# supranational/sppark

Measured on AMD Instinct MI355X. Metric: MSM points/sec (BLS12-381 G1, 2^26 points), higher is better.
Workload: dtype u32

## Files before the change

sppark_amd/csrc/msm/msm_driver.hpp:

```cpp
#pragma once
#include "msm_kernels.hpp"
#include "msm_coop_kernels.hpp"
#include "msm_plan.hpp"
#include "../ec/jacobian_host.hpp"
#include "../util/runtime.hpp"
#include <algorithm>
#include <cmath>
#include <map>
#include <mutex>
#include <vector>

namespace sppark_amd {

template<class FD, class FH, class FRp>
class msm_t {
public:
    typedef FD fp_d;
    static constexpr bool G2_COOP_BUILT = field_is_internal<FD>::value && !field_is_montx<FD>::value;
    typedef mont_dev<FRp> fr_d;
    typedef FH fp_h;
    typedef typename xyzz_dev<fp_d>::mem_t bucket_t;
    typedef jacobian_host<fp_h> point_t;
    static constexpr int STD_WORDS = sizeof(FH) / 4;
    static constexpr size_t FP_BYTES = sizeof(FH);
// ... 248 lines not shown
    {
        if (tune.wbits) return std::min(26u, std::max(8u, tune.wbits));
        unsigned w = 0; double best = 0;
        for (unsigned c = 8; c <= 26; c++) {
            const double cost = (double)((FRp::NBITS - 1) / c + 1) * (double)np + 3.0 * (double)((size_t)1 << (c - 1));
            if (w == 0 || cost < best) { best = cost; w = c; }
        }
        return w;
    }
    void preload(const void* points, size_t np, size_t ffi_affine_sz, bool fixed_base = false)
    {
        HIP_OK(hipSetDevice(gpu->hip_id));
        HIP_OK(hipStreamSynchronize(stream));
        join_default_stream();
        if (np != 0 && (points == nullptr || ffi_affine_sz < 2 * FP_BYTES || np > (1u << 31))) HIP_OK(hipErrorInvalidValue);
        if (np != 0 && fixed_base && !MONTX) HIP_OK(hipErrorNotSupported);
        if (np != 0 && fixed_base && (tune.wbits || np >= FIXED_BASE_MIN)
            && (size_t)((FRp::NBITS - 1) / fixed_base_width(np) + 1) * np >= ((size_t)1 << 31)) HIP_OK(hipErrorInvalidValue);
        if (pre_points) { HIP_OK(hipFree(pre_points)); pre_points = nullptr; pre_n = pre_stride = 0; }
        pre_fb_wbits = pre_fb_nwins = 0;
        if (np == 0) return;
        if (fixed_base && !MONTX) HIP_OK(hipErrorNotSupported);
        if (fixed_base && !tune.wbits && np < FIXED_BASE_MIN) fixed_base = false;
        unsigned fb_w = 0, fb_nw = 1;
        if (fixed_base) {
            fb_w = fixed_base_width(np);
            fb_nw = (FRp::NBITS - 1) / fb_w + 1;
            fb_w = FRp::NBITS / fb_nw + (FRp::NBITS % fb_nw ? 1 : 0);
            if ((size_t)fb_nw * np >= ((size_t)1 << 31)) HIP_OK(hipErrorInvalidValue);
        }
        if (points == nullptr || ffi_affine_sz < 2 * FP_BYTES || np > (1u << 31)) HIP_OK(hipErrorInvalidValue);
        struct dev_buf {
            unsigned char* p = nullptr;
            ~dev_buf() { if (p) (void)hipFree(p); }
        } staging;
        try {
            if constexpr (INTERNAL) {
                const unsigned char* src = (const unsigned char*)points;
                if (!is_device_pointer(points)) {
                    HIP_OK(hipMalloc((void**)&staging.p, np * ffi_affine_sz));
                    HIP_OK(hipMemcpyAsync(staging.p, points, np * ffi_affine_sz, hipMemcpyHostToDevice, stream));
                    src = staging.p;
                }
                HIP_OK(dev_scratch_pool::malloc_or_drain((void**)&pre_points, (size_t)fb_nw * np * conv_stride()));
                launch_convert(pre_points, src, (unsigned)np, ffi_affine_sz);
                if constexpr (MONTX) if (fixed_base) {
                    hipLaunchKernelGGL(k_fixed_base_table<fp_d>, dim3((unsigned)((np + 255) / 256)), dim3(256), 0, stream,
                                       pre_points, (unsigned)np, fb_nw, (unsigned)FRp::NBITS);
                    HIP_OK(hipGetLastError());
                }
            } else {
                HIP_OK(hipMalloc((void**)&pre_points, np * ffi_affine_sz));
                HIP_OK(hipMemcpyAsync(pre_points, points, np * ffi_affine_sz,
                                      is_device_pointer(points) ? hipMemcpyDeviceToDevice : hipMemcpyHostToDevice, stream));
            }
            HIP_OK(hipStreamSynchronize(stream));
        } catch (...) {
            if (pre_points) { (void)hipFree(pre_points); pre_points = nullptr; }
            throw;
        }
        pre_n = np; pre_stride = ffi_affine_sz;
        if (fixed_base) { pre_fb_wbits = fb_w; pre_fb_nwins = fb_nw; }
    }
    unsigned fixed_base_windows() const { return pre_fb_nwins; }
    size_t preloaded() const { return pre_n; }

private:
    void launch_convert(unsigned char* dst, const unsigned char* src, unsigned n, size_t stride, hipStream_t on = nullptr)
    {
        if constexpr (INTERNAL) {
            if (on == nullptr) on = stream;
            unsigned grid = (n + 255) / 256;
            if constexpr (MONTX) {
                if ((stride == 2 * FP_BYTES || stride == 2 * FP_BYTES + 8) && ((size_t)src & 15) == 0 && tune.join != 6) {
                    if (stride == 2 * FP_BYTES) hipLaunchKernelGGL((k_convert_points_staged<fp_d, false>), dim3(grid), dim3(256), 0, on, dst, src, n);
                    else                        hipLaunchKernelGGL((k_convert_points_staged<fp_d, true>), dim3(grid), dim3(256), 0, on, dst, src, n);
                    HIP_OK(hipGetLastError());
                    return;
                }
            }
            if (stride > 2 * FP_BYTES) hipLaunchKernelGGL((k_convert_points<fp_d, true>), dim3(grid), dim3(256), 0, on, dst, src, n, (unsigned)stride);
            else                       hipLaunchKernelGGL((k_convert_points<fp_d, false>), dim3(grid), dim3(256), 0, on, dst, src, n, (unsigned)stride);
            HIP_OK(hipGetLastError());
        }
    }

    size_t choose_chunk(size_t n, size_t stage_per_point) const
    {
        size_t chunk = n;
        if (tune.chunk) chunk = std::min(n, std::max<size_t>(tune.chunk, 1));
        else if (stage_per_point && n > ((size_t)1 << 21)) {
            chunk = std::min<size_t>(std::max<size_t>(n / 4, (size_t)1 << 20), (size_t)1 << 24);
        }
        auto need = [&](size_t c) {
            return make_layout(make_plan(c, FRp::NBITS, tune), true).total + 2 * c * stage_per_point + 1024;
        };
        size_t limit = tune.max_scratch;
        if (!limit) {
            const bool blob_ok = make_layout(make_plan(chunk, FRp::NBITS, tune), true).total <= blob_sz;
            const bool stage_ok = stage_per_point == 0 || 2 * (chunk * stage_per_point + 512) <= stage_sz;
            if (blob_ok && stage_ok) return chunk;
            size_t free_b = 0, total_b = 0;
            if (hipMemGetInfo(&free_b, &total_b) != hipSuccess) { (void)hipGetLastError(); return chunk; }
            limit = free_b - (free_b >> 5) + blob_sz + stage_sz;
        }
        while (need(chunk) > limit && chunk > 4096) chunk = (chunk + 1) / 2;
        return chunk;
    }

    std::vector<size_t> chunk_bounds(size_t n, size_t chunk) const
    {
        std::vector<size_t> b{0};
        for (size_t lo = chunk; lo < n; lo += chunk) b.push_back(lo);
        b.push_back(n);
        return b;
    }

    void sort_group(hipStream_t ss, const msm_plan& p, const layout& l, unsigned b, unsigned w0, unsigned wn,
                    const u32* d_scalars, bool mont, unsigned fb_n = 0, unsigned fb_nwins = 0)
    {
        u32* digits = (u32*)(blob + l.digits[b]);
        u32* sorted = (u32*)(blob + l.sorted[b]);
        u32* H = (u32*)(blob + l.H[b]);
        u32* tot = (u32*)(blob + l.tot[b]);
        u32* off = (u32*)(blob + l.off[b]);
        void* partA = blob + l.partA[b];
        u32* offA = (u32*)(blob + l.offA[b]);
        const bool packed = p.IB != 0;
        unsigned ngp = 1; while (ngp < p.NG) ngp <<= 1;
        const partA_fmt fmt{H, p.IB, p.SH, ngp, p.nslabs};
        const unsigned nlong = p.nbits % p.nwins, sf = nlong == 0 ? wn : (nlong > w0 ? std::min(wn, nlong - w0) : 0u);
        if (fb_n) {
            unsigned grid = std::min<unsigned>((fb_n + 255) / 256, 256 * 16);
            hipLaunchKernelGGL(k_breakdown<fr_d>, dim3(grid), dim3(256), 0, ss,
                               digits, d_scalars, fb_n, fb_nwins, (unsigned)FRp::NBITS, (int)mont, 0u, fb_nwins);
        } else {
            unsigned grid = std::min<unsigned>((p.n + 255) / 256, 256 * 16);
            hipLaunchKernelGGL(k_breakdown<fr_d>, dim3(grid), dim3(256), 0, ss,
                               digits, d_scalars, p.n, p.nwins, p.nbits, (int)mont, w0, wn);
        }
        HIP_OK(hipGetLastError());
        size_t ldsA = (size_t)p.NA * 4, ldsB = ((size_t)1 << p.LB) * 4 + SORT_NT * 4 + (size_t)SORTB_STAGE * 4 + PARTA_MAX_GROUPS * 4;
        if (ldsA > 65536) { lds_attr((const void*)k_histA, ldsA); lds_attr(packed ? (const void*)k_scatterA<true> : (const void*)k_scatterA<false>, ldsA); }
        if (ldsB > 65536) lds_attr(packed ? (const void*)k_sortB<true> : (const void*)k_sortB<false>, ldsB);
        hipLaunchKernelGGL(k_histA, dim3(p.nslabs, wn), dim3(SORT_NT), ldsA, ss,
                           H, digits, p.n, p.nslabs, p.slab_sz, p.NA, p.LB, sf);
        HIP_OK(hipGetLastError());
        size_t na_total = (size_t)wn * p.NA;
        hipLaunchKernelGGL(k_scan_slabs, dim3((unsigned)((na_total + 255) / 256)), dim3(256), 0, ss,
                           H, tot, p.nslabs, p.NA, wn);
        HIP_OK(hipGetLastError());
        hipLaunchKernelGGL(k_scan_parts, dim3(wn), dim3(1024), 0, ss, offA, tot, p.NA);
        HIP_OK(hipGetLastError());
        if (p.NA <= SCATA_MAX_NA && p.LB < 16) {
            const size_t ldsS = scatterA_staged_lds(p.NA);
            lds_attr(packed ? (const void*)k_scatterA_staged<true> : (const void*)k_scatterA_staged<false>, ldsS);
            if (packed) hipLaunchKernelGGL(k_scatterA_staged<true>, dim3(p.nslabs, wn), dim3(SORT_NT), ldsS, ss,
                                           (u32*)partA, digits, H, offA, p.n, p.nslabs, p.slab_sz, p.NA, p.LB, sf, p.IB);
            else        hipLaunchKernelGGL(k_scatterA_staged<false>, dim3(p.nslabs, wn), dim3(SORT_NT), ldsS, ss,
                                           (uint2*)partA, digits, H, offA, p.n, p.nslabs, p.slab_sz, p.NA, p.LB, sf, p.IB);
        } else {
            if (packed) hipLaunchKernelGGL(k_scatterA<true>, dim3(p.nslabs, wn), dim3(SORT_NT), ldsA, ss,
                                           (u32*)partA, digits, H, offA, p.n, p.nslabs, p.slab_sz, p.NA, p.LB, sf, p.IB);
            else        hipLaunchKernelGGL(k_scatterA<false>, dim3(p.nslabs, wn), dim3(SORT_NT), ldsA, ss,
                                           (uint2*)partA, digits, H, offA, p.n, p.nslabs, p.slab_sz, p.NA, p.LB, sf, p.IB);
        }
        HIP_OK(hipGetLastError());
        const unsigned big = tune.big ? tune.big : p.big ? p.big : (1u << 18);
        u32* nbig = (u32*)(blob + l.bigl[b]); u32* blist = nbig + 1; u32* curB = (u32*)(blob + l.curB[b]);
        const bool may_be_big = p.n > big;
        if (may_be_big) HIP_OK(hipMemsetAsync(nbig, 0, 4, ss));
        if (packed) hipLaunchKernelGGL(k_sortB<true>, dim3(p.NA, wn), dim3(SORT_NT), ldsB, ss,
                                       sorted, off, (const u32*)partA, offA, p.n, p.NA, p.LB, sf, big, fmt);
        else        hipLaunchKernelGGL(k_sortB<false>, dim3(p.NA, wn), dim3(SORT_NT), ldsB, ss,
                                       sorted, off, (const uint2*)partA, offA, p.n, p.NA, p.LB, sf, big, fmt);
        HIP_OK(hipGetLastError());
        if (!may_be_big) return;
        hipLaunchKernelGGL(k_big_find, dim3((p.NA * wn + 255) / 256), dim3(256), 0, ss,
                           nbig, blist, off, offA, p.NA, p.LB, sf, wn, big);
        size_t ldsBig = ((size_t)1 << p.LB) * 4;
        const size_t avg = (size_t)p.n / p.NA;
        const unsigned split = avg > big / 2 ? (unsigned)std::min<size_t>(SORTB_SPLIT, avg / (BIG_STAGE / 2) + 1) : SORTB_SPLIT;
        if (packed) hipLaunchKernelGGL(k_big_hist<true>, dim3(1024), dim3(1024), ldsBig, ss, off, (const u32*)partA, offA, nbig, blist, p.n, p.NA, p.LB, sf, split);
        else        hipLaunchKernelGGL(k_big_hist<false>, dim3(1024), dim3(1024), ldsBig, ss, off, (const uint2*)partA, offA, nbig, blist, p.n, p.NA, p.LB, sf, split);
        hipLaunchKernelGGL(k_big_scan, dim3(p.NA > 64 && avg > big / 2 ? 1024 : 64), dim3(1024), 0, ss, off, curB, offA, nbig, blist, p.NA, p.LB, sf);
        const size_t ldsSc = big_scatter_lds(p.LB);
        if (ldsSc > 65536) lds_attr(packed ? (const void*)k_big_scatter<true> : (const void*)k_big_scatter<false>, ldsSc);
        if (packed) hipLaunchKernelGGL(k_big_scatter<true>, dim3(1024), dim3(1024), ldsSc, ss, sorted, curB, (const u32*)partA, offA, nbig, blist, p.n, p.NA, p.LB, sf, split, fmt);
        else        hipLaunchKernelGGL(k_big_scatter<false>, dim3(1024), dim3(1024), ldsSc, ss, sorted, curB, (const uint2*)partA, offA, nbig, blist, p.n, p.NA, p.LB, sf, split, fmt);
        HIP_OK(hipGetLastError());
    }

    void enqueue(const msm_plan& p, const layout& l, const unsigned char* d_points, size_t stride, bool preconverted,
                 const u32* d_scalars, bool mont, std_bucket_t* h_out, bool first_timed, unsigned fb_n = 0, unsigned fb_nwins = 0,
                 bool redo = false, bool may_defer = false)
    {
        const bool flagged = !preconverted && stride > 2 * FP_BYTES;
        const bool multi = p.G > 1;
        if (multi) need_aux();
        if (timing && first_timed && !redo) { need_tev(2 + 2 * p.G); HIP_OK(hipEventRecord(tev[0], stream)); }
        if (multi) {
            HIP_OK(hipEventRecord(ev_fork, stream));
            HIP_OK(hipStreamWaitEvent(aux, ev_fork, 0));
        }
        bucket_t* buckets = (bucket_t*)(blob + l.buckets);
        u32* keyA = (u32*)(blob + l.keyA); bucket_t* ptA = (bucket_t*)(blob + l.ptA);
        u32* keyB = (u32*)(blob + l.keyB); bucket_t* ptB = (bucket_t*)(blob + l.ptB);
        if (multi && !redo) HIP_OK(hipMemsetAsync(buckets, 0, (size_t)p.nwins * p.NB * sizeof(bucket_t), stream));

        for (unsigned g = 0; g < p.G && !redo; g++, gseq++) {
            const unsigned b = multi ? (gseq & 1) : 0, w0 = g * p.wpg, wn = std::min(p.wpg, p.nwins - w0);
            if (g == 0) {
                sort_group(stream, p, l, b, w0, wn, d_scalars, mont, fb_n, fb_nwins);
                if (INTERNAL && !preconverted) {
                    launch_convert(blob + l.conv, d_points, p.n, stride);
                    d_points = blob + l.conv;
                }
            } else {
                if (gseq >= 2) HIP_OK(hipStreamWaitEvent(aux, ev_accdone[b], 0));
                sort_group(aux, p, l, b, w0, wn, d_scalars, mont);
                HIP_OK(hipEventRecord(ev_sorted[b], aux));
                HIP_OK(hipStreamWaitEvent(stream, ev_sorted[b], 0));
            }
            if (timing && first_timed) HIP_OK(hipEventRecord(tev[2 + 2 * g], stream));
            {
                const u32* sorted = (const u32*)(blob + l.sorted[b]);
                const u32* off = (const u32*)(blob + l.off[b]);
                dim3 grid((p.chunks_per_win + 255) / 256, wn);
                bool by_pairs = false;
                if constexpr (G2_COOP_BUILT) {
                    if (tune.g2_coop == 1 || (tune.g2_coop == 0 && fp_d::NL >= 14)) {
                        by_pairs = true;
                        dim3 grid2((p.chunks_per_win + 63) / 64, wn);
                        hipLaunchKernelGGL((k_accumulate_g2c<fp_d>), grid2, dim3(G2C_NT), 0, stream,
                                           buckets, keyA, ptA, d_points, (unsigned)stride, sorted, off,
                                           p.n, p.NB, p.L, p.chunks_per_win, w0);
                    }
                }
                if (by_pairs) {}
                else if (flagged)
                    hipLaunchKernelGGL((k_accumulate<fp_d, true>), grid, dim3(256), 0, stream,
                                       buckets, keyA, ptA, d_points, (unsigned)stride, sorted, off,
                                       p.n, p.NB, p.L, p.chunks_per_win, w0);
                else
                    hipLaunchKernelGGL((k_accumulate<fp_d, false>), grid, dim3(256), 0, stream,
                                       buckets, keyA, ptA, d_points, (unsigned)stride, sorted, off,
                                       p.n, p.NB, p.L, p.chunks_per_win, w0);
                HIP_OK(hipGetLastError());
            }
            if (timing && first_timed) HIP_OK(hipEventRecord(tev[3 + 2 * g], stream));
            if (multi) HIP_OK(hipEventRecord(ev_accdone[b], stream));
        }

        const unsigned piece_cm = may_defer ? piece_tree_cmax(p, multi, fb_n) : 0;
        piece_pending = false;
        bool small_sums = false;
        if constexpr (MONTX)
            small_sums = !multi && fb_n == 0 && p.NB <= SMALL_SUMS_MAX_NB && p.NB >= 2 && tune.K1 == 0 && tune.top == 0 && tune.K == 0
                         && tune.join != 3 && tune.join != 4;
        bool flag_with_sums = false;
        if constexpr (MONTX) flag_with_sums = small_sums && (piece_cm != 0 || redo);
        if (flag_with_sums && !d_pflag) {
            HIP_OK(hipMalloc((void**)&d_pflag, 64));
            HIP_OK(hipMemsetAsync(d_pflag, 0, 64, stream));
        }
        if (piece_cm && !redo) {
            u32* flag = flag_with_sums ? d_pflag : (u32*)(blob + l.flag);
            if (!flag_with_sums) HIP_OK(hipMemsetAsync(flag, 0, 4, stream));
            const u32* off = (const u32*)(blob + l.off[0]);
            unsigned t_fused = ~0u;
            if constexpr (MONTX) if (tune.join != 4 && tune.join != 8)
                t_fused = piece_tail_t0((size_t)p.nwins * p.NB, piece_cm, tune.join >= 16 ? (size_t)1 << (tune.join - 16) : PIECE_FUSE_MAX);
            for (unsigned t = 0; (piece_cm >> (t + 1)) >= 1; t++) {
                const unsigned last = (piece_cm >> (t + 2)) == 0;
                const size_t nthr = (size_t)p.nwins * p.NB * (piece_cm >> (t + 1));
                if constexpr (MONTX) if (t == t_fused) {
                    const unsigned lgGB = piece_tail_lgGB(piece_cm, t);
                    const size_t nwg = (((size_t)p.nwins * p.NB) + ((size_t)1 << lgGB) - 1) >> lgGB;
                    hipLaunchKernelGGL(k_piece_tail_coop<fp_d>, dim3((unsigned)nwg), dim3(COOP_NT), 0, stream,
                                       buckets, keyA, ptA, off, p.NB, p.L, p.chunks_per_win, p.nwins, piece_cm, t, lgGB, flag);
                    HIP_OK(hipGetLastError());
                    break;
                }
                bool coop = false;
                if constexpr (MONTX) coop = nthr <= COOP_LEVEL_MAX && tune.join != 4;
                if constexpr (MONTX) {
                    if (coop) hipLaunchKernelGGL(k_piece_level_coop<fp_d>, dim3((unsigned)((nthr + 63) / 64)), dim3(COOP_NT), 0, stream,
                                                 buckets, keyA, ptA, off, p.NB, p.L, p.chunks_per_win, p.nwins, piece_cm, t, last, flag);
                }
                if (!coop) hipLaunchKernelGGL(k_piece_level<fp_d>, dim3((unsigned)((nthr + 255) / 256)), dim3(256), 0, stream,
                                              buckets, keyA, ptA, off, p.NB, p.L, p.chunks_per_win, p.nwins, piece_cm, t, last, flag);
                HIP_OK(hipGetLastError());
            }
            if (!h_flag) HIP_OK(hipHostMalloc((void**)&h_flag, 64, hipHostMallocDefault));
            if (!flag_with_sums) HIP_OK(hipMemcpyAsync(h_flag, flag, 4, hipMemcpyDeviceToHost, stream));
            h_flag_cur = flag_with_sums ? reinterpret_cast<const u32*>(h_out + p.nwins) : h_flag;
            piece_pending = true;
        }
        if (!piece_pending) {
            size_t nrec = (size_t)2 * p.nwins * p.chunks_per_win;
            u32* ik = keyA; bucket_t* ip = ptA; u32* ok = keyB; bucket_t* op = ptB;
            const u32* skip = nullptr;
            if (tune.join != 1 && !redo && (size_t)p.n / p.NB <= (size_t)4 * p.L) {
                u32* keyC = (u32*)(blob + l.keyC); u32* flag = (u32*)(blob + l.flag);
                HIP_OK(hipMemsetAsync(flag, 0, 4, stream));
                const size_t nthr = nrec / 2 + 1;
                hipLaunchKernelGGL(k_join_runs<fp_d>, dim3((unsigned)((nthr + 255) / 256)), dim3(256), 0, stream,
// ... 387 lines not shown
```

sppark_amd/csrc/msm/msm_sort_kernels.hpp:

```cpp
#pragma once
#include "../ff/mont_dev.hpp"
#include "msm_sort_records.hpp"

namespace sppark_amd {

static constexpr unsigned SORT_NT = 1024;
#define SORT_VGPRS 32
static constexpr int SORTB_UNROLL = 4;
static constexpr int SORTB_PER = 18;
static constexpr unsigned SORTB_STAGE = SORTB_PER * SORT_NT;

__host__ __device__ inline unsigned window_lb(unsigned LB, unsigned w, unsigned short_from)
{   return (w >= short_from && LB) ? LB - 1 : LB;   }

SPPARK_DEVFN u32 block_scan_excl(u32 s, u32* wsum, u32* total)
{
    const unsigned lane = threadIdx.x & 63, wave = threadIdx.x >> 6;
    u32 incl = s;
    #pragma unroll
    for (int dlt = 1; dlt < 64; dlt <<= 1) { u32 v = __shfl_up(incl, dlt); if (lane >= (unsigned)dlt) incl += v; }
    if (lane == 63) wsum[wave] = incl;
    __syncthreads();
    u32 wv = lane < 16 ? wsum[lane] : 0, before = lane < wave ? wv : 0, tot = wv;
    #pragma unroll
    for (int m = 1; m < 16; m <<= 1) { before += __shfl_xor(before, m); tot += __shfl_xor(tot, m); }
    before = __shfl(before, 0); *total = __shfl(tot, 0);
    __syncthreads();
    return before + incl - s;
}

__global__ __launch_bounds__(SORT_NT) __attribute__((amdgpu_num_vgpr(SORT_VGPRS)))
void k_histA(u32* __restrict__ H, const u32* __restrict__ digits, unsigned n,
             unsigned nslabs, unsigned slab_sz, unsigned NA, unsigned LBL, unsigned short_from)
{
    extern __shared__ u32 lds_cnt[];
    const unsigned slab = blockIdx.x, w = blockIdx.y, LB = window_lb(LBL, w, short_from);
    for (unsigned b = threadIdx.x; b < NA; b += blockDim.x) lds_cnt[b] = 0;
    __syncthreads();

    const unsigned lo = slab * slab_sz, hi = min(n, lo + slab_sz);
    const u32* dig = digits + (size_t)w * n;
    for (unsigned i = lo + threadIdx.x; i < hi; i += 4 * blockDim.x) {
        u32 d[4];
        #pragma unroll
        for (int u = 0; u < 4; u++) { unsigned j = i + u * blockDim.x; d[u] = j < hi ? dig[j] : 0; }
        #pragma unroll
        for (int u = 0; u < 4; u++) if (d[u]) atomicAdd(&lds_cnt[((d[u] & 0x7fffffffu) - 1) >> LB], 1u);
    }
    __syncthreads();

    u32* out = H + ((size_t)w * nslabs + slab) * NA;
    for (unsigned b = threadIdx.x; b < NA; b += blockDim.x) out[b] = lds_cnt[b];
}

__global__ __launch_bounds__(256)
void k_scan_slabs(u32* __restrict__ H, u32* __restrict__ tot, unsigned nslabs, unsigned NA, unsigned nwins)
{
    const size_t id = (size_t)blockIdx.x * 256 + threadIdx.x;
    if (id >= (size_t)nwins * NA) return;
    const unsigned w = id / NA, b = id % NA;
    u32 run = 0;
    for (unsigned s = 0; s < nslabs; s++) {
        u32* p = H + ((size_t)w * nslabs + s) * NA + b;
        u32 t = *p; *p = run; run += t;
    }
    tot[id] = run;
}

__global__ __launch_bounds__(1024)
void k_scan_parts(u32* __restrict__ offA, const u32* __restrict__ tot, unsigned NA)
{
    __shared__ u32 part[1024];
    const unsigned w = blockIdx.x, tid = threadIdx.x;
    const unsigned per = (NA + 1023) / 1024;
    const unsigned lo = min(NA, tid * per), hi = min(NA, lo + per);
    const u32* t = tot + (size_t)w * NA;
    u32 sum = 0;
    for (unsigned b = lo; b < hi; b++) sum += t[b];
    part[tid] = sum;
    __syncthreads();
    for (unsigned d = 1; d < 1024; d <<= 1) {
        u32 v = tid >= d ? part[tid - d] : 0;
        __syncthreads();
        part[tid] += v;
        __syncthreads();
    }
    u32 run = part[tid] - sum;
    u32* o = offA + (size_t)w * (NA + 1);
    for (unsigned b = lo; b < hi; b++) { o[b] = run; run += t[b]; }
    if (tid == 1023) o[NA] = part[1023];
}

template<bool PK>
__global__ __launch_bounds__(SORT_NT) __attribute__((amdgpu_num_vgpr(SORT_VGPRS)))
void k_scatterA(typename recA<PK>::type* __restrict__ partA, const u32* __restrict__ digits,
                const u32* __restrict__ H, const u32* __restrict__ offA,
                unsigned n, unsigned nslabs, unsigned slab_sz, unsigned NA, unsigned LBL, unsigned short_from, unsigned IB)
{
    extern __shared__ u32 lds_cur[];
    const unsigned slab = blockIdx.x, w = blockIdx.y, LB = window_lb(LBL, w, short_from);
    const u32* h = H + ((size_t)w * nslabs + slab) * NA;
    const u32* o = offA + (size_t)w * (NA + 1);
    for (unsigned b = threadIdx.x; b < NA; b += blockDim.x) lds_cur[b] = h[b] + o[b];
    __syncthreads();

    const unsigned lo = slab * slab_sz, hi = min(n, lo + slab_sz);
    const u32* dig = digits + (size_t)w * n;
    typename recA<PK>::type* dst = partA + (size_t)w * n;
    const u32 lomask = (1u << LB) - 1;
    for (unsigned i = lo + threadIdx.x; i < hi; i += 4 * blockDim.x) {
        u32 d[4];
        #pragma unroll
        for (int u = 0; u < 4; u++) { unsigned j = i + u * blockDim.x; d[u] = j < hi ? dig[j] : 0; }
        #pragma unroll
        for (int u = 0; u < 4; u++) {
            if (d[u]) {
                u32 k = (d[u] & 0x7fffffffu) - 1;
                u32 pos = atomicAdd(&lds_cur[k >> LB], 1u);
                dst[pos] = recA<PK>::make((i + u * blockDim.x) | (d[u] & 0x80000000u), k & lomask, LBL, IB);
            }
        }
    }
}

static constexpr int SCATA_PER = 14;
static constexpr unsigned SCATA_TILE = SCATA_PER * SORT_NT;
static constexpr unsigned SCATA_MAX_NA = 4 * SORT_NT;
static inline size_t scatterA_staged_lds(unsigned NA) { return (size_t)NA * 8 + 64 + (size_t)SCATA_TILE * 8; }

SPPARK_DEVFN void wait_vmem()
{
#if defined(__HIP_DEVICE_COMPILE__)
    __builtin_amdgcn_s_waitcnt(0x0f70);
#endif
}
SPPARK_DEVFN void lds_barrier()
{
#if defined(__HIP_DEVICE_COMPILE__)
    asm volatile("s_waitcnt lgkmcnt(0)\n\ts_barrier" ::: "memory");
#endif
}

template<bool PK>
__global__ __launch_bounds__(SORT_NT)
void k_scatterA_staged(typename recA<PK>::type* __restrict__ partA, const u32* __restrict__ digits,
                       const u32* __restrict__ H, const u32* __restrict__ offA,
                       unsigned n, unsigned nslabs, unsigned slab_sz, unsigned NA, unsigned LBL, unsigned short_from, unsigned IB)
{
    extern __shared__ u32 lds_sa[];
    constexpr unsigned NT = SORT_NT;
    u32* cnt = lds_sa;
    u32* G = cnt + NA;
    u32* wsum = G + NA;
    uint2* stage = reinterpret_cast<uint2*>(wsum + 16);
    const unsigned slab = blockIdx.x, w = blockIdx.y, tid = threadIdx.x, lane = tid & 63, wave = tid >> 6;
    const unsigned LB = window_lb(LBL, w, short_from);
    const u32* h = H + ((size_t)w * nslabs + slab) * NA;
    const u32* o = offA + (size_t)w * (NA + 1);
    u32 cur[4];
    #pragma unroll
    for (int i = 0; i < 4; i++) { unsigned b = 4 * tid + i; cur[i] = b < NA ? h[b] + o[b] : 0; if (b < NA) cnt[b] = 0; }

    const unsigned lo = slab * slab_sz, hi = min(n, lo + slab_sz);
    const u32* dig = digits + (size_t)w * n;
    typename recA<PK>::type* dst = partA + (size_t)w * n;
    const u32 lomask = (1u << LB) - 1;
    u32 d[SCATA_PER], dn[SCATA_PER];
    #pragma unroll
    for (int u = 0; u < SCATA_PER; u++) { unsigned j = lo + u * NT + tid; dn[u] = j < hi ? dig[j] : 0; }
    __syncthreads();

    wait_vmem();
    #pragma unroll
    for (int u = 0; u < SCATA_PER; u++) d[u] = dn[u];
    for (unsigned t0 = lo; t0 < hi; t0 += SCATA_TILE) {
        #pragma unroll
        for (int u = 0; u < SCATA_PER; u++) { unsigned j = t0 + SCATA_TILE + u * NT + tid; dn[u] = j < hi ? dig[j] : 0; }
        #pragma unroll
        for (int u = 0; u < SCATA_PER; u++) if (d[u]) atomicAdd(&cnt[((d[u] & 0x7fffffffu) - 1) >> LB], 1u);
        lds_barrier();
        u32 c[4], s = 0;
        #pragma unroll
        for (int i = 0; i < 4; i++) { unsigned b = 4 * tid + i; c[i] = b < NA ? cnt[b] : 0; s += c[i]; }
        u32 incl = s;
        #pragma unroll
        for (int dlt = 1; dlt < 64; dlt <<= 1) { u32 v = __shfl_up(incl, dlt); if (lane >= (unsigned)dlt) incl += v; }
        if (lane == 63) wsum[wave] = incl;
        lds_barrier();
        u32 wv = lane < 16 ? wsum[lane] : 0, before = lane < wave ? wv : 0, total = wv;
        #pragma unroll
        for (int m = 1; m < 16; m <<= 1) { before += __shfl_xor(before, m); total += __shfl_xor(total, m); }
        before = __shfl(before, 0); total = __shfl(total, 0);
        u32 run = before + incl - s;
        #pragma unroll
        for (int i = 0; i < 4; i++) {
            unsigned b = 4 * tid + i;
            if (b < NA) { cnt[b] = run; G[b] = cur[i] - run; }
            cur[i] += c[i]; run += c[i];
        }
        lds_barrier();
        #pragma unroll
        for (int u = 0; u < SCATA_PER; u++) {
            if (d[u]) {
                u32 k = (d[u] & 0x7fffffffu) - 1, p = k >> LB;
                u32 pos = atomicAdd(&cnt[p], 1u);
                stage[pos] = make_uint2((t0 + u * NT + tid) | (d[u] & 0x80000000u), (p << 16) | (k & lomask));
            }
        }
        lds_barrier();
        wait_vmem();
        #pragma unroll
        for (int u = 0; u < SCATA_PER; u++) d[u] = dn[u];
        #pragma unroll
        for (int i = 0; i < 4; i++) { unsigned b = 4 * tid + i; if (b < NA) cnt[b] = 0; }
        #pragma unroll
        for (int u = 0; u < SCATA_PER; u++) {
            unsigned e = u * NT + tid;
            if (e < total) { uint2 v = stage[e]; dst[G[v.y >> 16] + e] = recA<PK>::make(v.x, v.y & 0xffffu, LBL, IB); }
        }
        lds_barrier();
    }
}

template<bool PK>
__global__ __launch_bounds__(SORT_NT) __attribute__((amdgpu_num_vgpr(64)))
void k_sortB(u32* __restrict__ sorted, u32* __restrict__ off, const typename recA<PK>::type* __restrict__ partA,
             const u32* __restrict__ offA, unsigned n, unsigned NA, unsigned LBL, unsigned short_from, unsigned big, partA_fmt fmt)
{
    extern __shared__ u32 lds[];
    typedef typename recA<PK>::type rec_t;
    constexpr unsigned NT = SORT_NT;
    const unsigned LB = window_lb(LBL, blockIdx.y, short_from);
    const size_t NB = (size_t)NA << LBL;
    const unsigned NL = 1u << LB;
    const u32 kmask = (1u << LBL) - 1;
    u32* cnt = lds;
    u32* part = lds + NL;
    u32* stage = part + NT;
    u32* bnd = stage + SORTB_STAGE;
    const unsigned khi = blockIdx.x, w = blockIdx.y, tid = threadIdx.x;
    const u32* oA = offA + (size_t)w * (NA + 1);
    const unsigned begin = oA[khi], end = oA[khi + 1];
    const rec_t* src = partA + (size_t)w * n;
    if (end - begin > big) {
        if (khi == NA - 1 && tid == 0) off[(size_t)w * (NB + 1) + NB] = end;
        if (LB != LBL) for (unsigned b = tid; b < NL; b += NT) off[(size_t)w * (NB + 1) + ((size_t)(NA + khi) << LB) + b] = oA[NA];
        return;
    }
    if (LB != LBL) for (unsigned b = tid; b < NL; b += NT) off[(size_t)w * (NB + 1) + ((size_t)(NA + khi) << LB) + b] = oA[NA];

    const bool in_regs = end - begin <= SORTB_STAGE;
    rec_t rr[SORTB_PER];
    for (unsigned b = tid; b < NL; b += NT) cnt[b] = 0;
    if (PK) partA_bounds(bnd, fmt, w, khi, NA, tid);
    __syncthreads();
    if (in_regs) {
        #pragma unroll
        for (int u = 0; u < SORTB_PER; u++) {
            unsigned j = begin + tid + u * NT;
            if (j < end) rr[u] = src[j];
        }
        #pragma unroll
        for (int u = 0; u < SORTB_PER; u++) if (begin + tid + u * NT < end) atomicAdd(&cnt[recA<PK>::key(rr[u], kmask)], 1u);
    } else {
        for (unsigned i = begin + tid; i < end; i += SORTB_UNROLL * NT) {
            rec_t r[SORTB_UNROLL];
            #pragma unroll
            for (int u = 0; u < SORTB_UNROLL; u++) { unsigned j = i + u * NT; if (j < end) r[u] = src[j]; }
            #pragma unroll
            for (int u = 0; u < SORTB_UNROLL; u++) if (i + u * NT < end) atomicAdd(&cnt[recA<PK>::key(r[u], kmask)], 1u);
        }
    }
    __syncthreads();

    const unsigned per = (NL + NT - 1) / NT;
    const unsigned lo = min(NL, tid * per), hi = min(NL, lo + per);
    u32 sum = 0;
    #pragma unroll 1
    for (unsigned b = lo; b < hi; b++) sum += cnt[b];
    u32 all;
    u32 run = begin + block_scan_excl(sum, part, &all);
    u32* o = off + (size_t)w * (NB + 1) + ((size_t)khi << LB);
    #pragma unroll 1
    for (unsigned b = lo; b < hi; b++) { u32 c = cnt[b]; cnt[b] = run; o[b] = run; run += c; }
    if (khi == NA - 1 && tid == 0) off[(size_t)w * (NB + 1) + NB] = end;
    __syncthreads();

    u32* dst = sorted + (size_t)w * n;
    if (in_regs) {
        #pragma unroll
        for (int u = 0; u < SORTB_PER; u++)
            if (begin + tid + u * NT < end)
                stage[atomicAdd(&cnt[recA<PK>::key(rr[u], kmask)], 1u) - begin] = recA<PK>::entry(rr[u], tid + u * NT, LBL, fmt, bnd);
        __syncthreads();
        for (unsigned i = tid; i < end - begin; i += NT) dst[begin + i] = stage[i];
        return;
    }
    for (unsigned i = begin + tid; i < end; i += SORTB_UNROLL * NT) {
        rec_t r[SORTB_UNROLL];
        #pragma unroll
        for (int u = 0; u < SORTB_UNROLL; u++) { unsigned j = i + u * NT; if (j < end) r[u] = src[j]; }
        #pragma unroll
        for (int u = 0; u < SORTB_UNROLL; u++) {
            if (i + u * NT < end) {
                u32 pos = atomicAdd(&cnt[recA<PK>::key(r[u], kmask)], 1u);
                dst[pos] = recA<PK>::entry(r[u], i + u * NT - begin, LBL, fmt, bnd);
            }
        }
    }
}

static constexpr unsigned SORTB_SPLIT = 64;
static constexpr int BIG_UNROLL = 4;

__global__ __launch_bounds__(256)
void k_big_find(u32* __restrict__ nbig, u32* __restrict__ list, u32* __restrict__ off,
                const u32* __restrict__ offA, unsigned NA, unsigned LBL, unsigned short_from, unsigned nwins, unsigned big)
{
    const unsigned id = blockIdx.x * blockDim.x + threadIdx.x;
    bool listed = false;
    if (id < NA * nwins) {
        const unsigned w = id / NA, khi = id % NA;
        const u32* oA = offA + (size_t)w * (NA + 1);
        listed = oA[khi + 1] - oA[khi] > big;
        if (listed) list[atomicAdd(nbig, 1u)] = id;
    }
    unsigned long long m = __ballot(listed);
    while (m) {
        const unsigned l = __builtin_ctzll(m); m &= m - 1;
        const unsigned pid = (id & ~63u) + l, w = pid / NA, khi = pid % NA, LB = window_lb(LBL, w, short_from);
        u32* o = off + (size_t)w * (((size_t)NA << LBL) + 1) + ((size_t)khi << LB);
        for (unsigned j = threadIdx.x & 63; j < (1u << LB); j += 64) o[j] = 0;
    }
}

__device__ inline bool big_slice(const u32* nbig, const u32* list, const u32* offA, unsigned NA, unsigned item, unsigned split,
                                 unsigned& w, unsigned& khi, unsigned& lo, unsigned& hi, unsigned& begin)
{
    const unsigned b = item / split, s = item % split;
    if (b >= *nbig) return false;
    w = list[b] / NA; khi = list[b] % NA;
    const u32* oA = offA + (size_t)w * (NA + 1);
    begin = oA[khi];
    const unsigned end = oA[khi + 1];
    const unsigned per = (end - begin + split - 1) / split;
    lo = min(end, begin + s * per); hi = min(end, lo + per);
    return true;
}

template<bool PK>
__global__ __launch_bounds__(1024)
void k_big_hist(u32* __restrict__ off, const typename recA<PK>::type* __restrict__ partA, const u32* __restrict__ offA,
                const u32* __restrict__ nbig, const u32* __restrict__ list, unsigned n, unsigned NA, unsigned LBL, unsigned short_from,
                unsigned split)
{
    extern __shared__ u32 lds[];
    const unsigned tid = threadIdx.x;
    const u32 kmask = (1u << LBL) - 1;
    for (unsigned item = blockIdx.x; ; item += gridDim.x) {
        unsigned w, khi, lo, hi, begin;
        if (!big_slice(nbig, list, offA, NA, item, split, w, khi, lo, hi, begin)) return;
        const unsigned LB = window_lb(LBL, w, short_from), NL = 1u << LB;
        for (unsigned j = tid; j < NL; j += 1024) lds[j] = 0;
        __syncthreads();
        const typename recA<PK>::type* src = partA + (size_t)w * n;
        for (unsigned i = lo + tid; i < hi; i += BIG_UNROLL * 1024) {
            u32 k[BIG_UNROLL];
            #pragma unroll
            for (int u = 0; u < BIG_UNROLL; u++) { unsigned j = i + u * 1024; k[u] = j < hi ? recA<PK>::key(src[j], kmask) : 0xffffffffu; }
            #pragma unroll
            for (int u = 0; u < BIG_UNROLL; u++) if (k[u] != 0xffffffffu) atomicAdd(&lds[k[u]], 1u);
        }
        __syncthreads();
// ... 117 lines not shown
```

Before: 517.3 million.

## Add tiled scatterA kernel processing double tiles with multi-pass LDS staging

Adds k_scatterA_tiled, which handles 28 digits per thread per tile (twice the staged kernel's tile) while keeping the same LDS stage size. Elements are ranked once per tile, and the stage is filled and flushed in up to two passes. This cuts the per-tile histogram, scan and barrier overhead relative to the amount of work, and keeps coalesced partitioned writes. The cost is higher register pressure from 28-element arrays plus extra passes and barriers. The new kernel is the default, and the old path can be selected with an env var in tuning builds.

```diff
diff --git a/sppark_amd/csrc/msm/msm_driver.hpp b/sppark_amd/csrc/msm/msm_driver.hpp
--- a/sppark_amd/csrc/msm/msm_driver.hpp
+++ b/sppark_amd/csrc/msm/msm_driver.hpp
@@ -424,7 +424,18 @@
         HIP_OK(hipGetLastError());
         hipLaunchKernelGGL(k_scan_parts, dim3(wn), dim3(1024), 0, ss, offA, tot, p.NA);
         HIP_OK(hipGetLastError());
-        if (p.NA <= SCATA_MAX_NA && p.LB < 16) {
+        bool tiled = true;
+#ifdef SPPARK_TUNING
+        if (const char* e = getenv("SPPARK_MSM_SCATTERA")) tiled = atoi(e) != 1;
+#endif
+        if (tiled && p.NA <= SCATA_MAX_NA && p.LB < 16) {
+            const size_t ldsS = scatterA_tiled_lds(p.NA);
+            lds_attr(packed ? (const void*)k_scatterA_tiled<true> : (const void*)k_scatterA_tiled<false>, ldsS);
+            if (packed) hipLaunchKernelGGL(k_scatterA_tiled<true>, dim3(p.nslabs, wn), dim3(SORT_NT), ldsS, ss,
+                                           (u32*)partA, digits, H, offA, p.n, p.nslabs, p.slab_sz, p.NA, p.LB, sf, p.IB);
+            else        hipLaunchKernelGGL(k_scatterA_tiled<false>, dim3(p.nslabs, wn), dim3(SORT_NT), ldsS, ss,
+                                           (uint2*)partA, digits, H, offA, p.n, p.nslabs, p.slab_sz, p.NA, p.LB, sf, p.IB);
+        } else if (p.NA <= SCATA_MAX_NA && p.LB < 16) {
             const size_t ldsS = scatterA_staged_lds(p.NA);
             lds_attr(packed ? (const void*)k_scatterA_staged<true> : (const void*)k_scatterA_staged<false>, ldsS);
             if (packed) hipLaunchKernelGGL(k_scatterA_staged<true>, dim3(p.nslabs, wn), dim3(SORT_NT), ldsS, ss,
diff --git a/sppark_amd/csrc/msm/msm_sort_kernels.hpp b/sppark_amd/csrc/msm/msm_sort_kernels.hpp
--- a/sppark_amd/csrc/msm/msm_sort_kernels.hpp
+++ b/sppark_amd/csrc/msm/msm_sort_kernels.hpp
@@ -1,17 +1,15 @@
 #pragma once
 #include "../ff/mont_dev.hpp"
 #include "msm_sort_records.hpp"
+#include "msm_sort_shape.hpp"
 
 namespace sppark_amd {
 
-static constexpr unsigned SORT_NT = 1024;
 #define SORT_VGPRS 32
 static constexpr int SORTB_UNROLL = 4;
 static constexpr int SORTB_PER = 18;
 static constexpr unsigned SORTB_STAGE = SORTB_PER * SORT_NT;
 
-__host__ __device__ inline unsigned window_lb(unsigned LB, unsigned w, unsigned short_from)
-{   return (w >= short_from && LB) ? LB - 1 : LB;   }
 
 SPPARK_DEVFN u32 block_scan_excl(u32 s, u32* wsum, u32* total)
 {
@@ -123,8 +121,6 @@
     }
 }
 
-static constexpr int SCATA_PER = 14;
-static constexpr unsigned SCATA_TILE = SCATA_PER * SORT_NT;
 static constexpr unsigned SCATA_MAX_NA = 4 * SORT_NT;
 static inline size_t scatterA_staged_lds(unsigned NA) { return (size_t)NA * 8 + 64 + (size_t)SCATA_TILE * 8; }
 
@@ -219,6 +215,113 @@
             if (e < total) { uint2 v = stage[e]; dst[G[v.y >> 16] + e] = recA<PK>::make(v.x, v.y & 0xffffu, LBL, IB); }
         }
         lds_barrier();
+    }
+}
+
+static inline size_t scatterA_tiled_lds(unsigned NA) { return (size_t)NA * 8 + 64 + (size_t)SCATA2_STAGE * 8; }
+
+template<bool PK>
+__global__ __launch_bounds__(SORT_NT)
+void k_scatterA_tiled(typename recA<PK>::type* __restrict__ partA, const u32* __restrict__ digits,
+                      const u32* __restrict__ H, const u32* __restrict__ offA,
+                      unsigned n, unsigned nslabs, unsigned slab_sz, unsigned NA, unsigned LBL, unsigned short_from, unsigned IB)
+{
+    extern __shared__ u32 lds_sa[];
+    constexpr unsigned NT = SORT_NT, S = SCATA2_STAGE;
+    u32* cnt = lds_sa;
+    u32* G = cnt + NA;
+    u32* wsum = G + NA;
+    uint2* stage = reinterpret_cast<uint2*>(wsum + 16);
+    const unsigned slab = blockIdx.x, w = blockIdx.y, tid = threadIdx.x, lane = tid & 63, wave = tid >> 6;
+    const unsigned LB = window_lb(LBL, w, short_from);
+    const u32* h = H + ((size_t)w * nslabs + slab) * NA;
+    const u32* o = offA + (size_t)w * (NA + 1);
+    u32 cur[4];
+    #pragma unroll
+    for (int i = 0; i < 4; i++) { unsigned b = 4 * tid + i; cur[i] = b < NA ? h[b] + o[b] : 0; if (b < NA) cnt[b] = 0; }
+
+    const unsigned lo = slab * slab_sz, hi = min(n, lo + slab_sz);
+    const u32* dig = digits + (size_t)w * n;
+    typename recA<PK>::type* dst = partA + (size_t)w * n;
+    const u32 lomask = (1u << LB) - 1;
+    u32 d[SCATA2_PER], dn[SCATA2_PER], pos[SCATA2_PER];
+    #pragma unroll
+    for (int u = 0; u < SCATA2_PER; u++) { unsigned j = lo + u * NT + tid; dn[u] = j < hi ? dig[j] : 0; }
+    __syncthreads();
+
+    wait_vmem();
+    #pragma unroll
+    for (int u = 0; u < SCATA2_PER; u++) d[u] = dn[u];
+    for (unsigned t0 = lo; t0 < hi; t0 += SCATA2_TILE) {
+        #pragma unroll
+        for (int u = 0; u < SCATA2_PER; u++) { unsigned j = t0 + SCATA2_TILE + u * NT + tid; dn[u] = j < hi ? dig[j] : 0; }
+        #pragma unroll
+        for (int u = 0; u < SCATA2_PER; u++) if (d[u]) atomicAdd(&cnt[((d[u] & 0x7fffffffu) - 1) >> LB], 1u);
+        lds_barrier();
+        u32 c[4], s = 0;
+        #pragma unroll
+        for (int i = 0; i < 4; i++) { unsigned b = 4 * tid + i; c[i] = b < NA ? cnt[b] : 0; s += c[i]; }
+        u32 incl = s;
+        #pragma unroll
+        for (int dlt = 1; dlt < 64; dlt <<= 1) { u32 v = __shfl_up(incl, dlt); if (lane >= (unsigned)dlt) incl += v; }
+        if (lane == 63) wsum[wave] = incl;
+        lds_barrier();
+        u32 wv = lane < 16 ? wsum[lane] : 0, before = lane < wave ? wv : 0, total = wv;
+        #pragma unroll
+        for (int m = 1; m < 16; m <<= 1) { before += __shfl_xor(before, m); total += __shfl_xor(total, m); }
+        before = __shfl(before, 0); total = __shfl(total, 0);
+        u32 run = before + incl - s;
+        #pragma unroll
+        for (int i = 0; i < 4; i++) {
+            unsigned b = 4 * tid + i;
+            if (b < NA) { cnt[b] = run; G[b] = cur[i] - run; }
+            cur[i] += c[i]; run += c[i];
+        }
+        lds_barrier();
+        #pragma unroll
+        for (int u = 0; u < SCATA2_PER; u++) {
+            pos[u] = 0xffffffffu;
+            if (d[u]) {
+                u32 k = (d[u] & 0x7fffffffu) - 1, p = k >> LB;
+                pos[u] = atomicAdd(&cnt[p], 1u);
+                if (pos[u] < S) stage[pos[u]] = make_uint2((t0 + u * NT + tid) | (d[u] & 0x80000000u), (p << 16) | (k & lomask));
+            }
+        }
+        if (total <= S) {
+            wait_vmem();
+            #pragma unroll
+            for (int u = 0; u < SCATA2_PER; u++) d[u] = dn[u];
+        }
+        lds_barrier();
+        #pragma unroll
+        for (int i = 0; i < 4; i++) { unsigned b = 4 * tid + i; if (b < NA) cnt[b] = 0; }
+        #pragma unroll
+        for (int q = 0; q < SCATA2_PASSES; q++) {
+            const unsigned base = q * S;
+            if (base >= total) break;
+            if (q > 0) {
+                #pragma unroll
+                for (int u = 0; u < SCATA2_PER; u++) {
+                    const u32 r = pos[u] - base;
+                    if (r < S) {
+                        u32 k = (d[u] & 0x7fffffffu) - 1, p = k >> LB;
+                        stage[r] = make_uint2((t0 + u * NT + tid) | (d[u] & 0x80000000u), (p << 16) | (k & lomask));
+                    }
+                }
+                if (base + S >= total) {
+                    wait_vmem();
+                    #pragma unroll
+                    for (int u = 0; u < SCATA2_PER; u++) d[u] = dn[u];
+                }
+                lds_barrier();
+            }
+            #pragma unroll
+            for (int u = 0; u < (int)(S / NT); u++) {
+                unsigned e = base + u * NT + tid;
+                if (e < total) { uint2 v = stage[e - base]; dst[G[v.y >> 16] + e] = recA<PK>::make(v.x, v.y & 0xffffu, LBL, IB); }
+            }
+            lds_barrier();
+        }
     }
 }
 
diff --git a/sppark_amd/csrc/msm/msm_sort_shape.hpp b/sppark_amd/csrc/msm/msm_sort_shape.hpp
--- /dev/null
+++ b/sppark_amd/csrc/msm/msm_sort_shape.hpp
@@ -0,0 +1,19 @@
+#pragma once
+#include <hip/hip_runtime.h>
+
+namespace sppark_amd {
+
+static constexpr unsigned SORT_NT = 1024;
+
+static constexpr int SCATA_PER = 14;
+static constexpr unsigned SCATA_TILE = SCATA_PER * SORT_NT;
+
+static constexpr int SCATA2_PER = 28;
+static constexpr unsigned SCATA2_TILE = SCATA2_PER * SORT_NT;
+static constexpr unsigned SCATA2_STAGE = SCATA_TILE;
+static constexpr int SCATA2_PASSES = (SCATA2_TILE + SCATA2_STAGE - 1) / SCATA2_STAGE;
+
+__host__ __device__ inline unsigned window_lb(unsigned LB, unsigned w, unsigned short_from)
+{   return (w >= short_from && LB) ? LB - 1 : LB;   }
+
+}
```

Result: no change. 518.6 million, median of 6 (+0.3%).
